# rcanut/nhwcodec

Hardware: AMD Instinct MI355X
Metric: encode Mpixels/s (512x512 RGB batch) (higher is better)
Workload: dtype int16

## Files before the change

### include/nhw_hip_debug.h

```cpp
#ifndef NHW_HIP_DEBUG_H
#define NHW_HIP_DEBUG_H

#include "nhw_hip.h"

#ifdef __cplusplus
extern "C" {
#endif

int nhw_debug_stop_after(nhw_enc *e, int stage);
int nhw_debug_front_fallback(nhw_enc *e, int on);
int nhw_debug_read(nhw_enc *e, int buf, int img, void *dst, size_t bytes);
int nhw_debug_hash(nhw_enc *e, int buf, size_t bytes, int n, void *d_out, void *stream);

int nhw_debug_fill(nhw_enc *e, int buf, int byte, size_t bytes, int n);

int nhw_debug_slice_order(nhw_enc *e, int mode);
int nhw_dec_debug_slice_order(nhw_dec *d, int mode);

int nhw_stage_chroma_loops(nhw_enc *e, int n, int comp, int form, void *stream);
int nhw_debug_write(nhw_enc *e, int buf, int img, const void *src, size_t bytes);

void nhw_dec_debug_stop_after(nhw_dec *d, int stage);
int  nhw_dec_debug_read(nhw_dec *d, int what, int img, void *dst, size_t bytes);
int  nhw_dec_debug_colour(int quality, const void *d_yuv, void *d_rgb, int n);

#ifdef __cplusplus
}
#endif
#endif
```

### nhwcodec_amd/__init__.py

```python
import ctypes
import numbers
import os

HERE = os.path.dirname(os.path.abspath(__file__))
LIB_PATH = os.path.join(HERE, "libnhwhip.so")
IMG_BYTES = 786432
OUT_STRIDE = 512 << 10
QUALITY_DEFAULT = 20
NHW_OK, NHW_E_QUALITY, NHW_E_CODEBOOK, NHW_E_SPACE, NHW_E_ARG, NHW_E_HIP, NHW_E_FORMAT = 0, -1, -2, -3, -4, -5, -6
NHW_E_BUDGET = -7
PEAK_SSE_NUMERATOR = 65025 * IMG_BYTES

P = ctypes.c_void_p


class Timing(ctypes.Structure):
    _fields_ = [(n, ctypes.c_float) for n in ("total_ms", "front_ms", "color_dwt_ms", "luma_ms", "chroma_ms", "entropy_ms")] + [("parts", ctypes.c_int), ("front_images", ctypes.c_int), ("prefilter_ms", ctypes.c_float)]


class FitStats(ctypes.Structure):
    _fields_ = [("rungs", ctypes.c_int), ("quality", ctypes.c_int * 23), ("images", ctypes.c_int * 23), ("total_ms", ctypes.c_float)]


class NhwError(RuntimeError):
# ... 10 lines not shown
    L.nhw_enc_create_ex.argtypes = [ctypes.c_int, ctypes.c_int, ctypes.c_uint, ctypes.POINTER(P)]
    L.nhw_enc_destroy.argtypes = [P]
    L.nhw_quality_supported.argtypes = [ctypes.c_int]
    L.nhw_enc_set_compat.argtypes = [P, ctypes.c_int]
    L.nhw_enc_batch_device.argtypes = [P, P, ctypes.c_int, ctypes.c_int, P, P, P, P]
    L.nhw_enc_batch.argtypes = [P, P, ctypes.c_int, ctypes.c_int, P, ctypes.c_size_t, P, P]
    L.nhw_synth_batch_device.argtypes = [P, P, ctypes.c_int, ctypes.c_uint32, P]
    L.nhw_enc_last_timing.argtypes = [P, ctypes.POINTER(Timing)]
    L.nhw_enc_synth_batch.argtypes = [P, ctypes.c_int, ctypes.c_uint32, ctypes.c_int, P, ctypes.c_size_t, P, P]
    L.nhw_host_alloc.restype = P
    L.nhw_host_alloc.argtypes = [ctypes.c_size_t]
    L.nhw_host_free.argtypes = [P]
    L.nhw_device_count.restype = ctypes.c_int
    L.nhw_enc_fit_batch_device.argtypes = [P, P, ctypes.c_int, P, P, ctypes.c_int, P, P, P, P, P]
    L.nhw_enc_fit_batch.argtypes = [P, P, ctypes.c_int, P, P, ctypes.c_int, P, ctypes.c_size_t, P, P, P]
    L.nhw_enc_last_fit_stats.argtypes = [P, ctypes.POINTER(FitStats)]
    L.nhw_sse_batch_device.argtypes = [P, P, ctypes.c_int, P, P]
    L.nhw_enc_fit_sse_batch_device.argtypes = [P, P, P, ctypes.c_int, P, P, ctypes.c_int, P, P, P, P, P, P]
    L.nhw_enc_fit_sse_batch.argtypes = [P, P, P, ctypes.c_int, P, P, ctypes.c_int, P, ctypes.c_size_t, P, P, P, P]
    L.nhw_stage_color.argtypes = [P, P, ctypes.c_int, ctypes.c_int, P, P, P, P]
    L.nhw_stage_prefilter.argtypes = [P, P, ctypes.c_int, ctypes.c_int, P]
    L.nhw_stage_chroma_l1.argtypes = [P, ctypes.c_int, P]
    L.nhw_stage_chroma_loops.argtypes = [P, ctypes.c_int, ctypes.c_int, ctypes.c_int, P]
    L.nhw_debug_write.argtypes = [P, ctypes.c_int, ctypes.c_int, P, ctypes.c_size_t]
    L.nhw_stage_analysis.argtypes = [P, P, P, ctypes.c_int, ctypes.c_size_t, ctypes.c_int, ctypes.c_int, ctypes.c_int, P]
    L.nhw_stage_synthesis.argtypes = [P, P, P, ctypes.c_int, ctypes.c_size_t, ctypes.c_int, ctypes.c_int, P]
    L.nhw_debug_slice_order.argtypes = [P, ctypes.c_int]
    L.nhw_dec_debug_slice_order.argtypes = [P, ctypes.c_int]
    L.nhw_picture_tiles.argtypes = [ctypes.c_uint32, ctypes.c_uint32]
    L.nhw_tile_pictures_device.argtypes = [P, ctypes.c_int, ctypes.c_int, ctypes.c_int, P, P]
    L.nhw_untile_pictures_device.argtypes = [P, P, ctypes.c_int, ctypes.c_int, ctypes.c_int, P]
    L.nhw_picture_info.argtypes = [P, ctypes.c_size_t, ctypes.POINTER(ctypes.c_uint32), ctypes.POINTER(ctypes.c_uint32)]
    L.nhw_enc_pictures.argtypes = [P, P, P, P, P, ctypes.c_int, ctypes.c_int, P, ctypes.c_size_t, P, P]
    L.nhw_dec_pictures.argtypes = [P, P, P, ctypes.c_int, P, P, P]
    L.nhw_sse_pictures_device.argtypes = [P, P, ctypes.c_int, ctypes.c_int, ctypes.c_int, P, P]
    L.nhw_enc_fit_pictures.argtypes = [P, P, P, P, P, ctypes.c_int, P, P, ctypes.c_int, P, ctypes.c_size_t, P, P, P]
    L.nhw_enc_fit_sse_pictures.argtypes = [P, P, P, P, P, P, ctypes.c_int, P, P, ctypes.c_int, P, ctypes.c_size_t, P, P, P, P]
    L.nhw_region_tiles.argtypes = [ctypes.c_uint32] * 6
    L.nhw_untile_regions_device.argtypes = [P, P, ctypes.c_int, ctypes.c_int, ctypes.c_int, P]
    L.nhw_dec_regions.argtypes = [P, P, P, ctypes.c_int, P, ctypes.c_int, P, P, P]
    L.nhw_dec_regions_to_device.argtypes = [P, P, P, ctypes.c_int, P, ctypes.c_int, P, P, P]
    L.nhw_dec_last_region_stats.argtypes = [P, ctypes.POINTER(ctypes.c_uint64), ctypes.POINTER(ctypes.c_uint64)]
    return L


_LIB = None
# ... 676 lines not shown
```

### nhwcodec_amd/csrc/nhw_dwt.h

```cpp
#ifndef NHW_DWT_H
#define NHW_DWT_H
#include <hip/hip_runtime.h>
#include <stdint.h>

__device__ __forceinline__ void lds_barrier() { asm volatile("s_waitcnt lgkmcnt(0)\n\ts_barrier" ::: "memory"); }

template <int S>
__device__ __forceinline__ void syn_pair(const int16_t *x, int st, int k, bool normalise, int *e_out, int *o_out)
{
	constexpr int M = S / 2;
	const int16_t *lo = x, *hi = x + M * st;
	const int l0 = lo[k * st], ln = (k + 1 < M) ? lo[(k + 1) * st] : l0;
	const int h0 = hi[k * st], hp = k > 0 ? hi[(k - 1) * st] : hi[0], hn = (k + 1 < M) ? hi[(k + 1) * st] : h0;
	int16_t e = (int16_t)(l0 << 3);
	int16_t o = (int16_t)((l0 + ln) << 2);
	e = (int16_t)(e - ((h0 + hp) << 1));
	o = (int16_t)(o + (6 * h0 - hp - hn));
	if (normalise) {
		if (e > 0) e = (int16_t)(e + 32);
		e >>= 6;
		if (o > 0) o = (int16_t)(o + 32);
		o >>= 6;
	}
	*e_out = e; *o_out = o;
// ... 29 lines not shown
typedef short s16x2 __attribute__((ext_vector_type(2)));
typedef unsigned short u16x2 __attribute__((ext_vector_type(2)));
__device__ __forceinline__ s16x2 as_s(uint32_t x) { return __builtin_bit_cast(s16x2, x); }
__device__ __forceinline__ u16x2 as_us(uint32_t x) { return __builtin_bit_cast(u16x2, x); }
__device__ __forceinline__ uint32_t as_w(s16x2 x) { return __builtin_bit_cast(uint32_t, x); }
__device__ __forceinline__ uint32_t as_w(u16x2 x) { return __builtin_bit_cast(uint32_t, x); }
__device__ __forceinline__ unsigned pk_add16(unsigned a, unsigned b)
{
	unsigned d;
	asm("v_pk_add_u16 %0, %1, %2" : "=v"(d) : "v"(a), "v"(b));
	return d;
}

__device__ __forceinline__ uint32_t pk_max_u16x(uint32_t a, uint32_t b) { uint32_t d; asm("v_pk_max_u16 %0, %1, %2" : "=v"(d) : "v"(a), "v"(b)); return d; }
__device__ __forceinline__ s16x2 pk_rnd_half_away(s16x2 v, int shift) { return (v + (s16x2)(short)(1 << (shift - 1)) + (v >> 15)) >> shift; }
__device__ __forceinline__ s16x2 pk_diffuse(s16x2 r)
{
	const s16x2 s = r >> 15, a = (r ^ s) - s;
	const s16x2 t = (s16x2)(a << 10) >> 10;
	const s16x2 d = (t + ((t >> 15) & (s16x2)(short)3)) >> 2;
	return (d ^ s) - s;
}

template <int PPL>
__device__ __forceinline__ void ana_row_pair(const uint32_t (&Dw)[PPL], int lane, int (&lo)[PPL], int (&hi)[PPL])
{
#pragma unroll
	for (int u = 0; u < PPL; u++) {
		uint32_t pv = (uint32_t)__builtin_amdgcn_update_dpp(0, (int)Dw[u], 0x138 , 0xF, 0xF, false);
		uint32_t nx = (uint32_t)__builtin_amdgcn_update_dpp(0, (int)Dw[u], 0x130 , 0xF, 0xF, false);
		if (u > 0) { const uint32_t seam = (uint32_t)__builtin_amdgcn_readlane((int)Dw[u > 0 ? u - 1 : 0], 63); if (lane == 0) pv = seam; }
		if (u + 1 < PPL) { const uint32_t seam = (uint32_t)__builtin_amdgcn_readlane((int)Dw[u + 1 < PPL ? u + 1 : u], 0); if (lane == 63) nx = seam; }
		else if (lane == 63) nx = Dw[u];
		const int e0 = (int16_t)(Dw[u] & 0xFFFF), o0 = (int)Dw[u] >> 16, e1 = (int16_t)(nx & 0xFFFF);
		int em1 = (int16_t)(pv & 0xFFFF), om1 = (int)pv >> 16;
		if (u == 0 && lane == 0) { em1 = e1; om1 = o0; }
		lo[u] = 6 * e0 + 2 * (om1 + o0) - (em1 + e1);
		hi[u] = (o0 << 1) - (e0 + e1);
	}
}

template <int PPL, int HLF, bool IN_RANGE = false >
__device__ __forceinline__ void ana_col_pair(const uint32_t (&Ew)[PPL], const uint32_t (&Ow)[PPL], bool left, int lane, int (&lo)[PPL][2], int (&hi)[PPL][2])
{
	bool wide = false;
	if (!IN_RANGE)
#pragma unroll
	for (int u = 0; u < PPL; u++) {
		const uint32_t mx = pk_max_u16x(pk_add16(Ew[u], 0x05140514u), pk_add16(Ow[u], 0x05140514u));
		wide |= (mx & 0xFFFFu) > 4300u || (mx >> 16) > 4300u;
	}
	if (IN_RANGE || !__any(wide)) {
		uint32_t rlast = 0;
#pragma unroll
		for (int u = 0; u < PPL; u++) {
			const int k = lane + 64 * u;
			uint32_t em = (uint32_t)__builtin_amdgcn_update_dpp(0, (int)Ew[u], 0x138, 0xF, 0xF, false), om = (uint32_t)__builtin_amdgcn_update_dpp(0, (int)Ow[u], 0x138, 0xF, 0xF, false);
			uint32_t en = (uint32_t)__builtin_amdgcn_update_dpp(0, (int)Ew[u], 0x130, 0xF, 0xF, false);
			if (u > 0) {
				const uint32_t se = (uint32_t)__builtin_amdgcn_readlane((int)Ew[u > 0 ? u - 1 : 0], 63), so_ = (uint32_t)__builtin_amdgcn_readlane((int)Ow[u > 0 ? u - 1 : 0], 63);
				if (lane == 0) { em = se; om = so_; }
			}
// ... 62 lines not shown
```

### nhwcodec_amd/csrc/nhw_enc.hip

```cpp
#include "nhw_enc.h"

thread_local std::string nhw_enc_err;
extern "C" const char *nhw_last_error(void) { return nhw_enc_err.c_str(); }

static const size_t k_buf_bytes[B_COUNT] = {
	 8 * Q,  8 * Q,  Q,  Q,  2 * Q,  2 * Q,
	 2 * Q,  2 * Q,  Q / 2,  Q / 2,  4 * Q,  2 * Q,
	 2 * Q,  4 * Q + 256,  8 * Q,  16,  512,  6 * Q,
	 24832,  16384,  16384 + 256,  32768,  16384,  32768,
	 8192,  2 * Q + 1024,  2 * Q + 256,  2 * Q + 1024,  2 * Q + 1024,  Q / 2,
	 Q + 64, 8192 + 64, 16384 + 64,  Q + 64, 8192 + 64, 16384 + 64,  Q + 64, 8192 + 64, 16384 + 64,
	 2 * Q + 1024, 16384 + 64, 16384 + 64,  2048 + 64,  8 * Q + 64,
	 512,  512,  320000,  768,  768,  16384 + 64,  16384 + 64,
	 131072,  131072,  5632,  256,  512,  16,  16,  (8 + 9 * 512) * 2,
	 Q / 2 + 256,  Q / 2,  Q / 4,  4 * Q,
	 Q / 4 + 256,  2 * Q,
	 2 * Q,  2 * Q,  Q / 2,  Q / 2,  Q,
	 320 * 512
};

static size_t round_up(size_t v, size_t a) { return (v + a - 1) / a * a; }

extern "C" int nhw_quality_supported(int quality) { return quality >= 1 && quality <= 23; }

// ... 119 lines not shown
	                    widen_in_analysis ? (comp ? plane8(ws, B_PV) : plane8(ws, B_PU)) : nullptr, ws.stride[B_PU], ws.dbg ? 0 : 2);
	if (low) nhw_launch_low_chroma_thin(cproc, cps, n, cs);
	STAGE_DONE();
	STAGE_DONE();
	if (!ws.dbg) {
		nhw_launch_chroma_loops(cproc, cps, cll1, ws.stride[B_CLL1] / 2, cl2save, ws.stride[B_CL2SAVE] / 2, plane8(ws, B_PU), ws.stride[B_PU], q, comp, ws.compat, n, cs);
		return 1;
	}
	nhw_launch_analysis(cjpeg, cproc, n, cps, H, H / 2, 1, cs);
	STAGE_DONE();
	nhw_launch_phase(PH_C2, ws, comp, out, d_sizes, d_status, cs);
	STAGE_DONE();
	nhw_launch_synthesis(cjpeg, cproc, n, cps, H, H / 2, cs);
	STAGE_DONE();
	nhw_launch_phase(PH_C3, ws, comp, out, d_sizes, d_status, cs);
	STAGE_DONE();
	nhw_launch_analysis(cjpeg, cproc, n, cps, H, H / 2, 1, cs, cl2save, ws.stride[B_CL2SAVE] / 2, H / 2, 1);
	STAGE_DONE();
	STAGE_DONE();
	nhw_launch_phase(PH_C4, ws, comp, out, d_sizes, d_status, cs);
	STAGE_DONE();
	nhw_launch_synthesis(cjpeg, cproc, n, cps, H, H / 2, cs);
	STAGE_DONE();
	return 1;
}

static int run_batch(nhw_enc *e, const NhwWs &ws_in, const void *d_bgr, int n, int quality, void *d_out, uint32_t *d_sizes, int32_t *d_status, hipStream_t s,
                     int timed ,
                     int what = 3 )
{
	NhwWs ws = ws_in;
	const int q = quality;
	const bool low = q <= 16;
	int16_t *jpeg = plane16(ws, B_JPEG), *proc = plane16(ws, B_PROC);
	int16_t *cjpeg = plane16(ws, B_CJPEG), *cproc = plane16(ws, B_CPROC);
	const size_t ps = ws.stride[B_JPEG] / 2, cps = ws.stride[B_CJPEG] / 2;
	uint8_t *out = (uint8_t *)d_out;

	e->low_parts_used = 1;
	int stage = 0;
	(void)n;
	if (what & 1) {
	if (timed == 1) HIPCHK(hipEventRecord(e->ev[EV_START], s));
	int16_t *yin = plane16(ws, B_KMAP);
	const size_t yin_stride = ws.stride[B_KMAP];
	if (low) {
// ... 23 lines not shown
	}
	STAGE_DONE();
	STAGE_DONE();
	if (timed == 1) HIPCHK(hipEventRecord(e->ev[EV_FRONT], s));
	if (!(what & 2)) { HIPCHK(hipGetLastError()); return NHW_OK; }
	}
	const bool fork = timed == 1 && what == 3 && !e->stop_after && e->chroma_fork;
	const bool fork_ll = fork && q > 13 && !ws.compat && e->ll_fork;
	ws.defer_verbatim = fork_ll;
	hipStream_t cs = fork ? e->part_stream[0] : s;
	ws.split_chroma = fork;
	auto chroma_head = [&](int comp) -> int { return chroma_head_launches(e, ws, comp, n, cs, stage); };
	auto chroma_tail = [&](int comp) -> int {
		nhw_launch_phase(PH_C5, ws, comp, out, d_sizes, d_status, cs);
		STAGE_DONE();
		return 1;
	};
#define CHROMA(call) do { const int rc_ = (call); if (rc_ != 1) return rc_; } while (0)
	if (fork) {
		HIPCHK(hipStreamWaitEvent(cs, !low || e->low_chroma == 0 ? e->ev[EV_FRONT] : (e->low_chroma == 2 && e->low_parts_used > 1) ? e->low_ev[low_ev_pass_a(e->low_parts_used - 1)] : e->ev[EV_COLOR], 0));
		CHROMA(chroma_head(0));
		CHROMA(chroma_head(1));
	}
	nhw_launch_analysis(jpeg, proc, n, ps, W, H, 1, s, nullptr, 0, 0, 0, nullptr, 0, 0, plane16(ws, B_LL1), ws.stride[B_LL1] / 2, H);
	STAGE_DONE();
	if (q > 6) {
	nhw_launch_phase(PH_L1, ws, 0, out, d_sizes, d_status, s);
	nhw_launch_wave(WV_DQ1, ws, s);
	STAGE_DONE();
	if (ws.dbg) {
	nhw_launch_synthesis(jpeg, proc, n, ps, W, H, s);
	STAGE_DONE();
	nhw_launch_phase(PH_L2, ws, 0, out, d_sizes, d_status, s);
	STAGE_DONE();
	} else nhw_launch_l2_recon(jpeg, proc, ps, plane16(ws, B_LL1), ws.stride[B_LL1] / 2, n, s);
	if (q > 12) nhw_launch_analysis(jpeg, proc, n, ps, W, H, 1, s, plane16(ws, B_L2SAVE), ws.stride[B_L2SAVE] / 2, H, 1);
	else nhw_launch_analysis(jpeg, proc, n, ps, W, H, 1, s);
	STAGE_DONE();
	}
	if (q <= 12) {
		nhw_launch_low_ll2(proc, ps, q, n, s);
		nhw_launch_copy_block(proc, ps, W, plane16(ws, B_L2SAVE), ws.stride[B_L2SAVE] / 2, H, H, H, n, s);
	}
	STAGE_DONE();
	nhw_launch_wave(WV_EMIT, ws, s);
	if (fork_ll) {
		HIPCHK(hipEventRecord(e->ll_ev[LL_EV_FORK], s));
		HIPCHK(hipStreamWaitEvent(e->ll_stream, e->ll_ev[LL_EV_FORK], 0));
		nhw_launch_phase(PH_L3, ws, 0, out, d_sizes, d_status, e->ll_stream);
		HIPCHK(hipEventRecord(e->ll_ev[LL_EV_DONE], e->ll_stream));
		HIPCHK(hipEventRecord(e->part_ev[PE_LUMA_LIST], e->ll_stream));
	} else {
	nhw_launch_phase(PH_L3, ws, 0, out, d_sizes, d_status, s);
	if (fork) HIPCHK(hipEventRecord(e->part_ev[PE_LUMA_LIST], s));
	}
	if (q > 12) {
	nhw_launch_wave(WV_DQ0, ws, s);
	STAGE_DONE();
	if (fork_ll) {
		HIPCHK(hipStreamWaitEvent(s, e->ll_ev[LL_EV_DONE], 0));
		nhw_launch_synthesis(jpeg, proc, n, ps, W, H, s, q <= 21 && !ws.dbg, ws.buf<uint16_t>(B_LLMEM, 0), ws.stride[B_LLMEM], &ws.buf<NhwMeta>(B_META, 0)->ll_mem_len, ws.stride[B_META]);
	} else
// ... 217 lines not shown
	HIPCHK(hipStreamWaitEvent(s, e->ev[EV_END], 0));
	int16_t *cjpeg = plane16(ws, B_CJPEG), *cproc = plane16(ws, B_CPROC), *cll1 = plane16(ws, B_CLL1), *cl2save = plane16(ws, B_CL2SAVE);
	const size_t cps = ws.stride[B_CJPEG] / 2;
	if (form == 0) {
		int stage = 0;
		const int rc = chroma_head_launches(e, ws, comp, n, s, stage);
		if (rc != 1) return rc;
	} else if (form == 1)
		nhw_launch_chroma_loops(cproc, cps, cll1, ws.stride[B_CLL1] / 2, cl2save, ws.stride[B_CL2SAVE] / 2, plane8(ws, B_PU), ws.stride[B_PU], ws.q, comp, ws.compat, n, s);
	else {
		const int k = form - 1;
		nhw_launch_analysis(cjpeg, cproc, n, cps, H, H / 2, 1, s, nullptr, 0, 0, 0, nullptr, 0, 0, cll1, ws.stride[B_CLL1] / 2, H / 2);
		if (k > 1) nhw_launch_phase(PH_C2, ws, comp, nullptr, nullptr, nullptr, s);
		if (k > 2) nhw_launch_synthesis(cjpeg, cproc, n, cps, H, H / 2, s);
		if (k > 3) nhw_launch_phase(PH_C3, ws, comp, nullptr, nullptr, nullptr, s);
		if (k > 4) nhw_launch_analysis(cjpeg, cproc, n, cps, H, H / 2, 1, s, cl2save, ws.stride[B_CL2SAVE] / 2, H / 2, 1);
		if (k > 5) nhw_launch_phase(PH_C4, ws, comp, nullptr, nullptr, nullptr, s);
		if (k > 6) nhw_launch_synthesis(cjpeg, cproc, n, cps, H, H / 2, s);
	}
	HIPCHK(hipGetLastError());
	return NHW_OK;
}

extern "C" int nhw_stage_synthesis(nhw_enc *e, void *d_jpeg, void *d_proc, int n_img, size_t plane_stride, int stride, int size, void *stream)
{
	if (!e || n_img < 1) return NHW_E_ARG;
	if (size != 256 && size != 128) { nhw_enc_err = "synthesis: transform size must be 256 or 128 (the encoder has no synthesis of size 512)"; return NHW_E_ARG; }
	HIPCHK(hipSetDevice(e->device));
	nhw_launch_synthesis((int16_t *)d_jpeg, (int16_t *)d_proc, n_img, plane_stride, stride, size, stream ? (hipStream_t)stream : e->own_stream);
	HIPCHK(hipGetLastError());
	return NHW_OK;
}

extern "C" int nhw_debug_front_fallback(nhw_enc *e, int on) { if (!e) return NHW_E_ARG; e->front_fallback = on; return NHW_OK; }
extern "C" int nhw_debug_stop_after(nhw_enc *e, int stage) { if (!e) return NHW_E_ARG; e->stop_after = stage; return NHW_OK; }
extern "C" int nhw_debug_slice_order(nhw_enc *e, int mode) { if (!e || mode < 0 || mode > 2) return NHW_E_ARG; e->slice_order = mode; return NHW_OK; }
__global__ __launch_bounds__(256) void k_debug_hash(const uint8_t *base, size_t stride, size_t words, unsigned long long *out)
{
	const uint32_t *p = reinterpret_cast<const uint32_t *>(base + (size_t)blockIdx.x * stride);
	unsigned long long h = 0;
	for (size_t i = threadIdx.x; i < words; i += 256) {
		unsigned long long x = ((unsigned long long)p[i] + 0x9E3779B97F4A7C15ull) * (2 * i + 1);
		x ^= x >> 29; x *= 0xBF58476D1CE4E5B9ull; x ^= x >> 32;
		h += x;
	}
	if (threadIdx.x == 0) out[blockIdx.x] = 0;
// ... 37 lines not shown
```

### nhwcodec_amd/csrc/nhw_host.h

```cpp
#ifndef NHW_HOST_H
#define NHW_HOST_H

#include <hip/hip_runtime.h>
#include <stdint.h>
#include <string>
#include <vector>

#include "../../include/nhw_hip.h"

struct NhwWs;

extern thread_local int nhw_slice_mode;

struct NhwSliceScope {
	int saved;
	explicit NhwSliceScope(int mode) : saved(nhw_slice_mode) { nhw_slice_mode = mode; }
	~NhwSliceScope() { nhw_slice_mode = saved; }
};

template <typename F> inline void nhw_slices(int nslices, F &&launch)
{
	if (nhw_slice_mode == 1) for (int i = 0; i < nslices; i++) launch(i);
	else if (nhw_slice_mode == 2) for (int i = nslices - 1; i >= 0; i--) launch(i);
	else launch(-1);
}

void nhw_launch_color(const uint8_t *bgr, int n, int q, int16_t *y, size_t y_stride, uint8_t *u, uint8_t *v, size_t c_stride, hipStream_t s);
void nhw_launch_analysis(int16_t *jpeg, int16_t *proc, int n, size_t plane_stride, int stride, int size, int final_level, hipStream_t s,
                         int16_t *save = nullptr, size_t save_plane = 0, int save_row = 0, int save_kind = 0, const uint8_t *src8 = nullptr, size_t src8_plane = 0, int drop_t = 0,
                         const int16_t *alt = nullptr, size_t alt_plane = 0, int alt_stride = 0);
void nhw_launch_synthesis(int16_t *jpeg, int16_t *proc, int n, size_t plane_stride, int stride, int size, hipStream_t s, int drop_nat = 0,
                          const uint16_t *verb_list = nullptr, size_t verb_list_stride = 0, const int *verb_len = nullptr, size_t verb_len_stride = 0);
void nhw_launch_synth(uint8_t *bgr, int n, uint32_t seed_base, hipStream_t s);
void nhw_launch_front_fused(const uint8_t *bgr, int q, uint8_t *pu, uint8_t *pv, size_t c_stride, const int16_t *y, size_t y_stride, int with_prefilter,
                            uint8_t *st, size_t s_stride, int16_t *proc, int16_t *jpeg, size_t plane_stride, int16_t *ll1, size_t ll1_stride,
                            int16_t *keep, size_t keep_stride, int n, hipStream_t s, int switches);
void nhw_launch_front_stale(const int16_t *y, size_t y_stride, const uint8_t *st, size_t s_stride, int16_t *stale, size_t stale_stride, int n, hipStream_t s);
int nhw_front_set_attrs(const char **where);
enum { PH_L1, PH_L2, PH_L3, PH_L4A, PH_C0, PH_C2, PH_C3, PH_C4, PH_C5, PH_FINAL, PH_L4B, PH_L4C, PH_L4D, PH_LLC, PH_L4C2 };
enum { WV_DQ1, WV_DQ0, WV_EMIT, WV_QUANT };
void nhw_launch_phase(int ph, const NhwWs &ws, int comp, uint8_t *out, uint32_t *sizes, int32_t *status, hipStream_t s);
void nhw_launch_wave(int ph, const NhwWs &ws, hipStream_t s);
void nhw_launch_l2_recon(int16_t *jpeg, const int16_t *proc, size_t plane_stride, int16_t *ll1, size_t ll1_stride, int n, hipStream_t s);
void nhw_launch_chroma_loops(int16_t *cproc, size_t plane_stride, int16_t *cll1, size_t ll1_stride, int16_t *cl2save, size_t save_stride,
                             const uint8_t *pu, size_t pu_stride, int q, int comp, int compat, int n, hipStream_t s);
void nhw_launch_copy_block(const int16_t *src, size_t src_plane, int src_row, int16_t *dst, size_t dst_plane, int dst_row, int rows, int cols, int n, hipStream_t s);
int nhw_tail_set_attrs(const char **where);
enum { LOW_EV_START = 0, LOW_EV_COUNT = 13 };
inline int low_ev_pass_a(int p) { return 1 + p; }
inline int low_ev_done(int parts, int p) { return 1 + parts + p; }
int nhw_launch_low_prefilter(const int16_t *src, size_t src_stride, int16_t *y, size_t y_stride, int16_t *km, size_t km_stride, uint8_t *so, size_t so_stride, uint8_t *chain, size_t chain_stride,
                             uint16_t *tab, size_t tab_stride, int q, int n, hipStream_t s, int force = 0, int parts = 1, hipStream_t *aux = nullptr, hipEvent_t *ev = nullptr);
void nhw_launch_low_prefilter_chroma(const uint8_t *src, size_t src_stride, int16_t *dst, size_t dst_stride, int q, int n, hipStream_t s);
void nhw_launch_low_chroma_thin(int16_t *plane, size_t plane_stride, int n, hipStream_t s);
void nhw_launch_low_ll2(int16_t *proc, size_t plane_stride, int q, int n, hipStream_t s);
void nhw_launch_low_stale(const int16_t *km, size_t km_stride, int16_t *stale, size_t stale_stride, int n, hipStream_t s);
void nhw_launch_fit_gather(const uint8_t *d_bgr, const int *idx, int m, uint8_t *staging, hipStream_t s);
void nhw_launch_fit_select(const int *idx, int m, const uint8_t *st_out, const uint32_t *st_sizes, const int32_t *st_status, const void *limit,
                           const int32_t *dec_status, const uint64_t *sse, int quality, int last, uint8_t *out, uint32_t *sizes, int32_t *status,
                           int32_t *qual, uint64_t *sse_out, uint8_t *open, hipStream_t s);
void nhw_launch_fit_compact(const uint8_t *open, const int *idx, int m, int *next, int *count, hipStream_t s);
hipError_t nhw_launch_sse(const uint8_t *a, const uint8_t *b, int n, uint64_t *sse, hipStream_t s);
hipError_t nhw_launch_tile_pad(const nhw_picture *d_pics, int n_pics, int tile0, int m, uint8_t *d_tiles, hipStream_t s);
hipError_t nhw_launch_untile_crop(const uint8_t *d_tiles, const nhw_picture *d_pics, int n_pics, int tile0, int m, hipStream_t s);
hipError_t nhw_launch_untile_region(const uint8_t *d_tiles, const nhw_region *d_regs, int n_regs, int tile0, int m, hipStream_t s);
hipError_t nhw_launch_sse_crop(const uint8_t *d_tiles, const nhw_picture *d_pics, int n_pics, int tile0, int m, uint64_t *d_sse, hipStream_t s);
// ... 22 lines not shown
```

### nhwcodec_amd/csrc/nhw_tail.hip

```cpp
#include "nhw_host.h"
#include "nhw_tail_par.h"
#include "nhw_dwt.h"

using namespace nhw;

#ifndef NHW_DENSE_STREAM
#define NHW_DENSE_STREAM 0
#endif

template <int PH>
__global__ __launch_bounds__(256) void k_phase(NhwWs ws, int comp, uint8_t *out, uint32_t *sizes, int32_t *status)
{
	__shared__ int sh_counts[2];
	__shared__ int sh_pos[2 * NT + 2];
	__shared__ uint32_t sh_z[4 * Q / 16 / 32 + 4];
	extern __shared__ __attribute__((aligned(16))) int16_t dyn_lds[];
	const int img = blockIdx.x, tid = threadIdx.x;
	Ctx c;
	ctx_load(&c, ws, img, comp);
	if (PH == PH_L1) luma_p1_par(&c, tid, sh_pos);
	else if (PH == PH_L2) luma_p2_par(&c, tid, dyn_lds);
	else if (PH == PH_L3) luma_p3_par(&c, tid, sh_pos, sh_counts, dyn_lds, ws.q <= 12 || ws.dbg != 0);
	else if (PH == PH_L4A) luma_p4a_par(&c, tid, dyn_lds);
	else if (PH == PH_L4B) luma_p4b_par(&c, tid, sh_pos, dyn_lds);
// ... 52 lines not shown
	if (img >= ws.n) return;
	Ctx c;
	ctx_load(&c, ws, img);
	if (PH == WV_DQ1) wave_dequant_sim_luma(&c, 1, lane, dq_lut, false, ws.dbg != 0);
	else if (PH == WV_DQ0) wave_dequant_sim_luma(&c, 0, lane, dq_lut, !ws.dbg, ws.dbg != 0);
	else if (PH == WV_QUANT) {
		__shared__ __attribute__((aligned(16))) uint8_t park[4][16 * QROW];
		__shared__ uint32_t lut[4][QLUT + 3];
		PROF_BEGIN(); wave_quantise_luma(&c, lane, park[threadIdx.x >> 6], lut[threadIdx.x >> 6], ws.q > 21 || ws.dbg, NHW_DENSE_STREAM || ws.dbg, !(ws.q > 21 || ws.dbg)); if (!lane) PROF(&c, 15);
	}
	else if (PH == WV_EMIT) { PROF_BEGIN(); wave_emit_ll2(&c, lane); if (!lane) PROF(&c, 4); }
}
void nhw_launch_wave(int ph, const NhwWs &ws, hipStream_t s)
{
	const dim3 g((ws.n + 3) / 4), b(256);
	switch (ph) {
	case WV_DQ1: k_wave<WV_DQ1><<<g, b, 0, s>>>(ws); break;
	case WV_DQ0: k_wave<WV_DQ0><<<g, b, 0, s>>>(ws); break;
	case WV_EMIT: k_wave<WV_EMIT><<<g, b, 0, s>>>(ws); break;
	case WV_QUANT: k_wave<WV_QUANT><<<g, b, 0, s>>>(ws); break;
	}
}

__global__ __launch_bounds__(1024) void k_l2_recon(int16_t *__restrict__ jpegb, const int16_t *__restrict__ procb, size_t plane_stride, int16_t *__restrict__ ll1b, size_t ll1_stride, int n)
{
	extern __shared__ __attribute__((aligned(16))) int16_t smem[];
	constexpr int S = H, LS = S + 2, HLF = S / 2, PPL = HLF / 64, NT_ = 1024, NPRE = S * (S / 8) / NT_;
	const int t = threadIdx.x, lane = t & 63, wv = t >> 6;
	int16_t *A = smem;
	int8_t *ytab = reinterpret_cast<int8_t *>(A + S * LS);
	if (t < PRECOMP_TAB) ytab[t] = (int8_t)precomp_pick(t / 11 - 12, t % 11 - 5);
	uint4 pre[NPRE];
	if ((int)blockIdx.x < n) {
		const int16_t *src = jpegb + (size_t)blockIdx.x * plane_stride;
#pragma unroll
		for (int u = 0; u < NPRE; u++) { const int v = t + u * NT_; pre[u] = *reinterpret_cast<const uint4 *>(src + (size_t)(v / (S / 8)) * W + 8 * (v % (S / 8))); }
	}
	for (int img = blockIdx.x; img < n; img += gridDim.x) {
		int16_t *jp = jpegb + (size_t)img * plane_stride, *o = ll1b + (size_t)img * ll1_stride;
		const int16_t *p = procb + (size_t)img * plane_stride;
#pragma unroll
		for (int u = 0; u < NPRE; u++) {
			const int v = t + u * NT_, row = v / (S / 8), c8 = v % (S / 8);
			uint32_t *d = reinterpret_cast<uint32_t *>(A + row * LS + 8 * c8);
			d[0] = pre[u].x; d[1] = pre[u].y; d[2] = pre[u].z; d[3] = pre[u].w;
		}
		lds_barrier();
		if (img + (int)gridDim.x < n) {
			const int16_t *src = jpegb + (size_t)(img + gridDim.x) * plane_stride;
#pragma unroll
			for (int u = 0; u < NPRE; u++) { const int v = t + u * NT_; pre[u] = *reinterpret_cast<const uint4 *>(src + (size_t)(v / (S / 8)) * W + 8 * (v % (S / 8))); }
		}
		const int r0 = wv * 16, c0 = 4 * lane;
		int side = 0;
		if (lane < 16) side = p[(size_t)(r0 + lane) * W - 1];
		else if (lane < 32) side = p[(size_t)(r0 + lane - 16) * W + H];
		else if (lane == 32) { side = o[(size_t)r0 * H - 1]; if (wv > 0) side = side > 14000 ? side - 16000 : side > 10000 ? side - 12000 : side; }
		else if (lane == 33) { side = o[(size_t)(r0 + 16) * H]; if (wv < 15) side = side > 14000 ? side - 16000 : side > 10000 ? side - 12000 : side; }
		for (int i = 0; i < 16; i++) {
			int16_t *x = A + (wv * 16 + i) * LS;
			int e[PPL], od[PPL];
#pragma unroll
			for (int u = 0; u < PPL; u++) syn_pair<S>(x, 1, lane + 64 * u, false, &e[u], &od[u]);
#pragma unroll
			for (int u = 0; u < PPL; u++) reinterpret_cast<uint32_t *>(x)[lane + 64 * u] = (uint32_t)(uint16_t)e[u] | ((uint32_t)(uint16_t)od[u] << 16);
		}
		lds_barrier();
		for (int i = 0; i < 16; i++) {
			int16_t *x = A + wv * 16 + i;
			int e[PPL], od[PPL];
#pragma unroll
			for (int u = 0; u < PPL; u++) syn_pair<S>(x, LS, lane + 64 * u, true, &e[u], &od[u]);
#pragma unroll
			for (int u = 0; u < PPL; u++) { const int k = lane + 64 * u; x[(2 * k) * LS] = (int16_t)e[u]; x[(2 * k + 1) * LS] = (int16_t)od[u]; }
		}
		lds_barrier();
		auto ll1_row = [&](int i) { return *reinterpret_cast<const uint2 *>(o + (size_t)(r0 + (i < 16 ? i : 15)) * H + c0); };
		auto untag = [](int v) { return v > 14000 ? v - 16000 : v > 10000 ? v - 12000 : v; };
		uint2 w0 = ll1_row(0), w1 = ll1_row(1), w2 = ll1_row(2), w3 = ll1_row(3);
#pragma unroll 1
		for (int i = 0; i < 16; i++) {
			const int r = r0 + i;
			int v[4];
			unpack4(w0, v);
			w0 = w1; w1 = w2; w2 = w3; w3 = ll1_row(i + 4);
			bool any = false;
#pragma unroll
			for (int k = 0; k < 4; k++) {
				const int step = v[k] > 14000 ? 1 : v[k] > 10000 ? -1 : 0;
				if (!step) continue;
// ... 21 lines not shown
			const int o_right = i == 15 ? __builtin_amdgcn_readlane(side, 33) : untag((int)(int16_t)(__builtin_amdgcn_readlane((int)w1.x, 0) & 0xFFFF));
			w0 = w1; w1 = w2; w2 = w3; w3 = ll1_row(i + 4);
#pragma unroll
			for (int k = 0; k < 4; k++) { ov[k] = untag(ov[k]); pv[k] = A[(c0 + k) * LS + r]; d[k] = (int16_t)(pv[k] - ov[k]); }
			const int p_left = __shfl(side, i), p_right = __shfl(side, 16 + i);
			const int my_edge = lane ? p_right - o_right : p_left - o_left;
			o_left = __builtin_amdgcn_readlane(ov[3], 63);
			const int sd = __shfl_down(d[0], 1), su = __shfl_up(d[3], 1);
			const int dn4 = lane < 63 ? sd : my_edge;
			const int first = lane ? su : my_edge;
			const int nb[4] = { precomp_right(d[1]), precomp_right(d[2]), precomp_right(d[3]), precomp_right(dn4) };
			int prev_in = first;
			for (;;) {
				int prev = prev_in;
#pragma unroll
				for (int k = 0; k < 4; k++) { st[k] = ytab[precomp_index(d[k], nb[k] + prev)]; prev = d[k] + st[k]; }
				int np = __shfl_up(prev, 1);
				if (!lane) np = first;
				if (!__any(np != prev_in)) break;
				prev_in = np;
			}
			uint2 w;
			w.x = (uint32_t)(uint16_t)(ov[0] + st[0]) | ((uint32_t)(uint16_t)(ov[1] + st[1]) << 16); w.y = (uint32_t)(uint16_t)(ov[2] + st[2]) | ((uint32_t)(uint16_t)(ov[3] + st[3]) << 16);
			*reinterpret_cast<uint2 *>(jp + (size_t)r * W + c0) = w;
		}
		lds_barrier();
	}
}
void nhw_launch_l2_recon(int16_t *jpeg, const int16_t *proc, size_t plane_stride, int16_t *ll1, size_t ll1_stride, int n, hipStream_t s)
{
	k_l2_recon<<<n < 256 ? n : 256, 1024, H * (H + 2) * sizeof(int16_t) + 288, s>>>(jpeg, proc, plane_stride, ll1, ll1_stride, n);
}

__global__ __launch_bounds__(512) __attribute__((amdgpu_waves_per_eu(8, 8))) void k_chroma_loops(int16_t *__restrict__ cprocb, size_t plane_stride, int16_t *__restrict__ cll1b, size_t ll1_stride,
                                                      int16_t *__restrict__ saveb, size_t save_stride, const uint8_t *__restrict__ pub, size_t pu_stride,
                                                      int q, int comp, int compat)
{
	constexpr int S = H / 2, LS = S + 2, HLF = S / 2;
	__shared__ __attribute__((aligned(16))) int16_t A[S * LS];
	const int t = threadIdx.x, lane = t & 63, wv = t >> 6, img = blockIdx.x, r0 = wv * 16;
	int16_t *p = cprocb + (size_t)img * plane_stride, *o = cll1b + (size_t)img * ll1_stride, *save = saveb + (size_t)img * save_stride;
	const uint8_t *pu = pub + (size_t)img * pu_stride;
	const int behind = compat ? (int16_t)(pu[32768] | (pu[32769] << 8)) : 0;
	auto ll1_row = [&](int i) { return reinterpret_cast<const uint32_t *>(o + (size_t)(r0 + (i < 16 ? i : 15)) * S)[lane]; };
	uint32_t w0 = ll1_row(0), w1 = ll1_row(1), w2 = ll1_row(2), w3 = ll1_row(3);
	int side = 0;
	if (lane < 16) side = p[(size_t)(r0 + lane) * H + S];
	else if (lane == 16) side = wv < 7 ? o[(size_t)(r0 + 16) * S] : behind;
	if (t == 0) o[Q >> 2] = (int16_t)behind;
	auto ana_row = [&](int16_t *x, uint32_t w) {
		const uint32_t Dw[1] = { w };
		int lo[1], hi[1];
		ana_row_pair<1>(Dw, lane, lo, hi);
		x[lane] = (int16_t)lo[0]; x[HLF + lane] = (int16_t)hi[0];
// ... 111 lines not shown

static size_t phase_lds(int ph)
{
	const size_t tile = (size_t)NT * TLS * sizeof(int16_t);
	switch (ph) {
	case PH_L2: return 3 * 32 * 33 + 32;
	case PH_L3: return LL_LDS_BYTES;
	case PH_LLC: return LLC_LDS_BYTES;
	case PH_FINAL: return PK_LDS_BYTES;
	case PH_L4A: return RF_LDS_BYTES > (NT + 2) * TLS * sizeof(int16_t) ? RF_LDS_BYTES : (size_t)(NT + 2) * TLS * sizeof(int16_t);
	case PH_L4B: return (size_t)(NT + 2) * TLS * sizeof(int16_t);
	case PH_L4C: return 0;
	case PH_L4D: return SL_LDS_BYTES;
	case PH_C5: return CQ_LDS_BYTES > 32 * 130 * 2 + (32 * 128 + 258) * 2 ? CQ_LDS_BYTES : 32 * 130 * 2 + (32 * 128 + 258) * 2;
	default: return 0;
	}
}

int nhw_tail_set_attrs(const char **where)
{
#define SETATTR(fn) do { const hipError_t e_ = hipFuncSetAttribute(reinterpret_cast<const void *>(&fn), hipFuncAttributeMaxDynamicSharedMemorySize, 100 << 10); \
                         if (e_ != hipSuccess) { *where = "hipFuncSetAttribute(" #fn ", MaxDynamicSharedMemorySize)"; return (int)e_; } } while (0)
	SETATTR(k_phase<PH_L1>); SETATTR(k_phase<PH_L2>); SETATTR(k_phase<PH_L3>); SETATTR(k_phase<PH_C5>);
	{ const hipError_t e_ = hipFuncSetAttribute(reinterpret_cast<const void *>(&k_l2_recon), hipFuncAttributeMaxDynamicSharedMemorySize, (int)(H * (H + 2) * sizeof(int16_t) + 288));
	  if (e_ != hipSuccess) { *where = "hipFuncSetAttribute(k_l2_recon, MaxDynamicSharedMemorySize)"; return (int)e_; } }
#undef SETATTR
	return 0;
}

void nhw_launch_phase(int ph, const NhwWs &ws, int comp, uint8_t *out, uint32_t *sizes, int32_t *status, hipStream_t s)
{
	const dim3 g(ws.n), b(256);
	const size_t lds = phase_lds(ph);
	switch (ph) {
	case PH_L1: k_phase<PH_L1><<<g, b, lds, s>>>(ws, comp, out, sizes, status); break;
	case PH_L2: k_phase<PH_L2><<<g, b, lds, s>>>(ws, comp, out, sizes, status); break;
	case PH_L3: k_phase<PH_L3><<<g, b, lds, s>>>(ws, comp, out, sizes, status); break;
	case PH_L4A: if (ws.q >= 17) k_l4a<<<g, b, lds, s>>>(ws); else k_phase<PH_L4A><<<g, b, lds, s>>>(ws, comp, out, sizes, status); break;
	case PH_L4B: k_phase<PH_L4B><<<g, b, lds, s>>>(ws, comp, out, sizes, status); break;
	case PH_L4C: k_phase<PH_L4C><<<g, b, lds, s>>>(ws, comp, out, sizes, status); break;
	case PH_L4D: if (NHW_DENSE_STREAM || ws.dbg) k_phase<PH_L4D><<<g, b, lds, s>>>(ws, comp, out, sizes, status); else k_y31<<<g, 512, lds, s>>>(ws); break;
	case PH_LLC: k_phase<PH_LLC><<<g, b, lds, s>>>(ws, comp, out, sizes, status); break;
	case PH_L4C2: k_phase<PH_L4C2><<<g, b, lds, s>>>(ws, comp, out, sizes, status); break;
	case PH_C0: k_phase<PH_C0><<<g, b, lds, s>>>(ws, comp, out, sizes, status); break;
	case PH_C2: k_phase<PH_C2><<<g, b, lds, s>>>(ws, comp, out, sizes, status); break;
	case PH_C3: k_phase<PH_C3><<<g, b, lds, s>>>(ws, comp, out, sizes, status); break;
	case PH_C4: k_phase<PH_C4><<<g, b, lds, s>>>(ws, comp, out, sizes, status); break;
	case PH_C5: k_phase<PH_C5><<<g, b, lds, s>>>(ws, comp, out, sizes, status); break;
// ... 11 lines not shown
```

Baseline: 60820.

## Fuse level-2 luma analysis into l2_recon kernel for high quality

For quality above 12, the L2 reconstruction kernel now also runs the level-1 row and column analysis on the reconstructed plane while it is still in LDS. It writes jpeg, proc and the L2 save buffer directly, so the separate analysis launch and its global-memory round trip are removed. Row analysis uses DPP lane shifts to get neighbouring pixels. The luma loop launch sequence moves into a helper, and a new stage entry point is added to benchmark variants. The change adds LDS work and barriers inside the recon kernel, and adds an unroll pragma to the inner synthesis loop.

```diff
diff --git a/include/nhw_hip_debug.h b/include/nhw_hip_debug.h
--- a/include/nhw_hip_debug.h
+++ b/include/nhw_hip_debug.h
@@ -19,6 +19,7 @@
 
 int nhw_stage_chroma_loops(nhw_enc *e, int n, int comp, int form, void *stream);
 int nhw_debug_write(nhw_enc *e, int buf, int img, const void *src, size_t bytes);
+int nhw_stage_luma_loop(nhw_enc *e, int n, int form, void *stream);
 
 void nhw_dec_debug_stop_after(nhw_dec *d, int stage);
 int  nhw_dec_debug_read(nhw_dec *d, int what, int img, void *dst, size_t bytes);
diff --git a/nhwcodec_amd/__init__.py b/nhwcodec_amd/__init__.py
--- a/nhwcodec_amd/__init__.py
+++ b/nhwcodec_amd/__init__.py
@@ -56,6 +56,7 @@
     L.nhw_stage_prefilter.argtypes = [P, P, ctypes.c_int, ctypes.c_int, P]
     L.nhw_stage_chroma_l1.argtypes = [P, ctypes.c_int, P]
     L.nhw_stage_chroma_loops.argtypes = [P, ctypes.c_int, ctypes.c_int, ctypes.c_int, P]
+    L.nhw_stage_luma_loop.argtypes = [P, ctypes.c_int, ctypes.c_int, P]
     L.nhw_debug_write.argtypes = [P, ctypes.c_int, ctypes.c_int, P, ctypes.c_size_t]
     L.nhw_stage_analysis.argtypes = [P, P, P, ctypes.c_int, ctypes.c_size_t, ctypes.c_int, ctypes.c_int, ctypes.c_int, P]
     L.nhw_stage_synthesis.argtypes = [P, P, P, ctypes.c_int, ctypes.c_size_t, ctypes.c_int, ctypes.c_int, P]
diff --git a/nhwcodec_amd/csrc/nhw_dwt.h b/nhwcodec_amd/csrc/nhw_dwt.h
--- a/nhwcodec_amd/csrc/nhw_dwt.h
+++ b/nhwcodec_amd/csrc/nhw_dwt.h
@@ -75,6 +75,15 @@
 	return (d ^ s) - s;
 }
 
+__device__ __forceinline__ void ana_row_taps(uint32_t d, uint32_t pv, uint32_t nx, bool first, int *lo, int *hi)
+{
+	const int e0 = (int16_t)(d & 0xFFFF), o0 = (int)d >> 16, e1 = (int16_t)(nx & 0xFFFF);
+	int em1 = (int16_t)(pv & 0xFFFF), om1 = (int)pv >> 16;
+	if (first) { em1 = e1; om1 = o0; }
+	*lo = 6 * e0 + 2 * (om1 + o0) - (em1 + e1);
+	*hi = (o0 << 1) - (e0 + e1);
+}
+
 template <int PPL>
 __device__ __forceinline__ void ana_row_pair(const uint32_t (&Dw)[PPL], int lane, int (&lo)[PPL], int (&hi)[PPL])
 {
@@ -85,12 +94,17 @@
 		if (u > 0) { const uint32_t seam = (uint32_t)__builtin_amdgcn_readlane((int)Dw[u > 0 ? u - 1 : 0], 63); if (lane == 0) pv = seam; }
 		if (u + 1 < PPL) { const uint32_t seam = (uint32_t)__builtin_amdgcn_readlane((int)Dw[u + 1 < PPL ? u + 1 : u], 0); if (lane == 63) nx = seam; }
 		else if (lane == 63) nx = Dw[u];
-		const int e0 = (int16_t)(Dw[u] & 0xFFFF), o0 = (int)Dw[u] >> 16, e1 = (int16_t)(nx & 0xFFFF);
-		int em1 = (int16_t)(pv & 0xFFFF), om1 = (int)pv >> 16;
-		if (u == 0 && lane == 0) { em1 = e1; om1 = o0; }
-		lo[u] = 6 * e0 + 2 * (om1 + o0) - (em1 + e1);
-		hi[u] = (o0 << 1) - (e0 + e1);
+		ana_row_taps(Dw[u], pv, nx, u == 0 && lane == 0, &lo[u], &hi[u]);
 	}
+}
+
+__device__ __forceinline__ void ana_row_quad(uint32_t a, uint32_t b, int lane, int (&lo)[2], int (&hi)[2])
+{
+	const uint32_t pv = (uint32_t)__builtin_amdgcn_update_dpp(0, (int)b, 0x138 , 0xF, 0xF, false);
+	uint32_t nx = (uint32_t)__builtin_amdgcn_update_dpp(0, (int)a, 0x130 , 0xF, 0xF, false);
+	if (lane == 63) nx = b;
+	ana_row_taps(a, pv, b, lane == 0, &lo[0], &hi[0]);
+	ana_row_taps(b, a, nx, false, &lo[1], &hi[1]);
 }
 
 template <int PPL, int HLF, bool IN_RANGE = false >
diff --git a/nhwcodec_amd/csrc/nhw_enc.hip b/nhwcodec_amd/csrc/nhw_enc.hip
--- a/nhwcodec_amd/csrc/nhw_enc.hip
+++ b/nhwcodec_amd/csrc/nhw_enc.hip
@@ -165,6 +165,32 @@
 	STAGE_DONE();
 	nhw_launch_synthesis(cjpeg, cproc, n, cps, H, H / 2, cs);
 	STAGE_DONE();
+	return 1;
+}
+
+static int luma_loop_launches(nhw_enc *e, const NhwWs &ws, int n, hipStream_t s, int &stage)
+{
+	const int q = ws.q;
+	int16_t *jpeg = plane16(ws, B_JPEG), *proc = plane16(ws, B_PROC);
+	const size_t ps = ws.stride[B_JPEG] / 2;
+	uint8_t *out = nullptr; uint32_t *d_sizes = nullptr; int32_t *d_status = nullptr;
+	nhw_launch_analysis(jpeg, proc, n, ps, W, H, 1, s, nullptr, 0, 0, 0, nullptr, 0, 0, plane16(ws, B_LL1), ws.stride[B_LL1] / 2, H);
+	STAGE_DONE();
+	if (q > 6) {
+	nhw_launch_phase(PH_L1, ws, 0, out, d_sizes, d_status, s);
+	nhw_launch_wave(WV_DQ1, ws, s);
+	STAGE_DONE();
+	if (ws.dbg) {
+	nhw_launch_synthesis(jpeg, proc, n, ps, W, H, s);
+	STAGE_DONE();
+	nhw_launch_phase(PH_L2, ws, 0, out, d_sizes, d_status, s);
+	STAGE_DONE();
+	} else nhw_launch_l2_recon(jpeg, proc, ps, plane16(ws, B_LL1), ws.stride[B_LL1] / 2, n, s,
+	                           q > 12 ? plane16(ws, B_L2SAVE) : nullptr, ws.stride[B_L2SAVE] / 2);
+	if (q <= 12) nhw_launch_analysis(jpeg, proc, n, ps, W, H, 1, s);
+	else if (ws.dbg) nhw_launch_analysis(jpeg, proc, n, ps, W, H, 1, s, plane16(ws, B_L2SAVE), ws.stride[B_L2SAVE] / 2, H, 1);
+	STAGE_DONE();
+	}
 	return 1;
 }
 
@@ -234,22 +260,7 @@
 		CHROMA(chroma_head(0));
 		CHROMA(chroma_head(1));
 	}
-	nhw_launch_analysis(jpeg, proc, n, ps, W, H, 1, s, nullptr, 0, 0, 0, nullptr, 0, 0, plane16(ws, B_LL1), ws.stride[B_LL1] / 2, H);
-	STAGE_DONE();
-	if (q > 6) {
-	nhw_launch_phase(PH_L1, ws, 0, out, d_sizes, d_status, s);
-	nhw_launch_wave(WV_DQ1, ws, s);
-	STAGE_DONE();
-	if (ws.dbg) {
-	nhw_launch_synthesis(jpeg, proc, n, ps, W, H, s);
-	STAGE_DONE();
-	nhw_launch_phase(PH_L2, ws, 0, out, d_sizes, d_status, s);
-	STAGE_DONE();
-	} else nhw_launch_l2_recon(jpeg, proc, ps, plane16(ws, B_LL1), ws.stride[B_LL1] / 2, n, s);
-	if (q > 12) nhw_launch_analysis(jpeg, proc, n, ps, W, H, 1, s, plane16(ws, B_L2SAVE), ws.stride[B_L2SAVE] / 2, H, 1);
-	else nhw_launch_analysis(jpeg, proc, n, ps, W, H, 1, s);
-	STAGE_DONE();
-	}
+	{ const int rc_ = luma_loop_launches(e, ws, n, s, stage); if (rc_ != 1) return rc_; }
 	if (q <= 12) {
 		nhw_launch_low_ll2(proc, ps, q, n, s);
 		nhw_launch_copy_block(proc, ps, W, plane16(ws, B_L2SAVE), ws.stride[B_L2SAVE] / 2, H, H, H, n, s);
@@ -513,6 +524,45 @@
 	return NHW_OK;
 }
 
+extern "C" int nhw_stage_luma_loop(nhw_enc *e, int n, int form, void *stream)
+{
+	if (!e || n < 1 || n > e->max_batch || form < 0 || form > 5) { nhw_enc_err = "bad argument"; return NHW_E_ARG; }
+	if (!e->timed || n > e->last_n || e->stop_after || e->last_q < 7) {
+		nhw_enc_err = "nhw_stage_luma_loop: needs a completed whole batch of >= n images at quality >= 7 and no debug stop";
+		return NHW_E_ARG;
+	}
+	HIPCHK(hipSetDevice(e->device));
+	NhwWs ws = e->ws;
+	ws.n = n; ws.q = e->last_q; ws.dbg = 0;
+	hipStream_t s = stream ? (hipStream_t)stream : e->own_stream;
+	HIPCHK(hipStreamWaitEvent(s, e->ev[EV_END], 0));
+	int16_t *jpeg = plane16(ws, B_JPEG), *proc = plane16(ws, B_PROC), *ll1 = plane16(ws, B_LL1), *l2save = plane16(ws, B_L2SAVE);
+	const size_t ps = ws.stride[B_JPEG] / 2;
+	const bool save = ws.q > 12;
+	if (form == 0) {
+		int stage = 0;
+		const int rc = luma_loop_launches(e, ws, n, s, stage);
+		if (rc != 1) return rc;
+	} else if (form == 1) {
+		nhw_launch_l2_recon(jpeg, proc, ps, ll1, ws.stride[B_LL1] / 2, n, s, save ? l2save : nullptr, ws.stride[B_L2SAVE] / 2);
+		if (!save) nhw_launch_analysis(jpeg, proc, n, ps, W, H, 1, s);
+	} else {
+		if (form == 3 || form == 4) {
+			nhw_launch_analysis(jpeg, proc, n, ps, W, H, 1, s, nullptr, 0, 0, 0, nullptr, 0, 0, ll1, ws.stride[B_LL1] / 2, H);
+			nhw_launch_phase(PH_L1, ws, 0, nullptr, nullptr, nullptr, s);
+			nhw_launch_wave(WV_DQ1, ws, s);
+		}
+		nhw_launch_synthesis(jpeg, proc, n, ps, W, H, s);
+		if (form < 4) {
+			nhw_launch_phase(PH_L2, ws, 0, nullptr, nullptr, nullptr, s);
+			if (save) nhw_launch_analysis(jpeg, proc, n, ps, W, H, 1, s, l2save, ws.stride[B_L2SAVE] / 2, H, 1);
+			else nhw_launch_analysis(jpeg, proc, n, ps, W, H, 1, s);
+		}
+	}
+	HIPCHK(hipGetLastError());
+	return NHW_OK;
+}
+
 extern "C" int nhw_stage_synthesis(nhw_enc *e, void *d_jpeg, void *d_proc, int n_img, size_t plane_stride, int stride, int size, void *stream)
 {
 	if (!e || n_img < 1) return NHW_E_ARG;
diff --git a/nhwcodec_amd/csrc/nhw_host.h b/nhwcodec_amd/csrc/nhw_host.h
--- a/nhwcodec_amd/csrc/nhw_host.h
+++ b/nhwcodec_amd/csrc/nhw_host.h
@@ -41,7 +41,7 @@
 enum { WV_DQ1, WV_DQ0, WV_EMIT, WV_QUANT };
 void nhw_launch_phase(int ph, const NhwWs &ws, int comp, uint8_t *out, uint32_t *sizes, int32_t *status, hipStream_t s);
 void nhw_launch_wave(int ph, const NhwWs &ws, hipStream_t s);
-void nhw_launch_l2_recon(int16_t *jpeg, const int16_t *proc, size_t plane_stride, int16_t *ll1, size_t ll1_stride, int n, hipStream_t s);
+void nhw_launch_l2_recon(int16_t *jpeg, int16_t *proc, size_t plane_stride, int16_t *ll1, size_t ll1_stride, int n, hipStream_t s, int16_t *l2save = nullptr, size_t save_stride = 0);
 void nhw_launch_chroma_loops(int16_t *cproc, size_t plane_stride, int16_t *cll1, size_t ll1_stride, int16_t *cl2save, size_t save_stride,
                              const uint8_t *pu, size_t pu_stride, int q, int comp, int compat, int n, hipStream_t s);
 void nhw_launch_copy_block(const int16_t *src, size_t src_plane, int src_row, int16_t *dst, size_t dst_plane, int dst_row, int rows, int cols, int n, hipStream_t s);
diff --git a/nhwcodec_amd/csrc/nhw_tail.hip b/nhwcodec_amd/csrc/nhw_tail.hip
--- a/nhwcodec_amd/csrc/nhw_tail.hip
+++ b/nhwcodec_amd/csrc/nhw_tail.hip
@@ -98,7 +98,9 @@
 	}
 }
 
-__global__ __launch_bounds__(1024) void k_l2_recon(int16_t *__restrict__ jpegb, const int16_t *__restrict__ procb, size_t plane_stride, int16_t *__restrict__ ll1b, size_t ll1_stride, int n)
+template <bool ANA>
+__global__ __launch_bounds__(1024) void k_l2_recon(int16_t *__restrict__ jpegb, int16_t *__restrict__ procb, size_t plane_stride, int16_t *__restrict__ ll1b, size_t ll1_stride, int n,
+                                                   int16_t *__restrict__ saveb, size_t save_stride)
 {
 	extern __shared__ __attribute__((aligned(16))) int16_t smem[];
 	constexpr int S = H, LS = S + 2, HLF = S / 2, PPL = HLF / 64, NT_ = 1024, NPRE = S * (S / 8) / NT_;
@@ -114,7 +116,7 @@
 	}
 	for (int img = blockIdx.x; img < n; img += gridDim.x) {
 		int16_t *jp = jpegb + (size_t)img * plane_stride, *o = ll1b + (size_t)img * ll1_stride;
-		const int16_t *p = procb + (size_t)img * plane_stride;
+		int16_t *p = procb + (size_t)img * plane_stride;
 #pragma unroll
 		for (int u = 0; u < NPRE; u++) {
 			const int v = t + u * NT_, row = v / (S / 8), c8 = v % (S / 8);
@@ -142,6 +144,7 @@
 			for (int u = 0; u < PPL; u++) reinterpret_cast<uint32_t *>(x)[lane + 64 * u] = (uint32_t)(uint16_t)e[u] | ((uint32_t)(uint16_t)od[u] << 16);
 		}
 		lds_barrier();
+#pragma unroll 4
 		for (int i = 0; i < 16; i++) {
 			int16_t *x = A + wv * 16 + i;
 			int e[PPL], od[PPL];
@@ -209,14 +212,52 @@
 			}
 			uint2 w;
 			w.x = (uint32_t)(uint16_t)(ov[0] + st[0]) | ((uint32_t)(uint16_t)(ov[1] + st[1]) << 16); w.y = (uint32_t)(uint16_t)(ov[2] + st[2]) | ((uint32_t)(uint16_t)(ov[3] + st[3]) << 16);
-			*reinterpret_cast<uint2 *>(jp + (size_t)r * W + c0) = w;
+			if (!ANA) *reinterpret_cast<uint2 *>(jp + (size_t)r * W + c0) = w;
+			else {
+				int lo[2], hi[2];
+				ana_row_quad(w.x, w.y, lane, lo, hi);
+				int16_t *x = A + (2 * lane) * LS + r;
+				x[0] = (int16_t)lo[0]; x[LS] = (int16_t)lo[1]; x[HLF * LS] = (int16_t)hi[0]; x[(HLF + 1) * LS] = (int16_t)hi[1];
+			}
+		}
+		if (ANA) {
+			lds_barrier();
+			int16_t *save = saveb + (size_t)img * save_stride;
+			const int rr = lane >> 5, c8 = lane & 31;
+#pragma unroll 1
+			for (int i = 0; i < 8; i++) {
+				const int c = r0 + 2 * i;
+				const uint32_t *g = reinterpret_cast<const uint32_t *>(A + (c + rr) * LS + 8 * c8);
+				*reinterpret_cast<uint4 *>(jp + (size_t)(c + rr) * W + 8 * c8) = make_uint4(g[0], g[1], g[2], g[3]);
+				uint32_t Ew[PPL], Ow[PPL];
+				int lo[PPL][2], hi[PPL][2];
+#pragma unroll
+				for (int u = 0; u < PPL; u++) {
+					const uint32_t a = reinterpret_cast<const uint32_t *>(A + c * LS)[lane + 64 * u], b = reinterpret_cast<const uint32_t *>(A + (c + 1) * LS)[lane + 64 * u];
+					Ew[u] = (a & 0xFFFFu) | (b << 16); Ow[u] = (a >> 16) | (b & 0xFFFF0000u);
+				}
+				ana_col_pair<PPL, HLF>(Ew, Ow, c < HLF, lane, lo, hi);
+				asm volatile("" ::: "memory");
+#pragma unroll
+				for (int h = 0; h < 2; h++) {
+					int16_t *x = A + (c + h) * LS;
+#pragma unroll
+					for (int u = 0; u < PPL; u++) { x[lane + 64 * u] = (int16_t)lo[u][h]; x[HLF + lane + 64 * u] = (int16_t)hi[u][h]; }
+				}
+				asm volatile("" ::: "memory");
+				const uint4 w = make_uint4(g[0], g[1], g[2], g[3]);
+				*reinterpret_cast<uint4 *>(p + (size_t)(c + rr) * W + 8 * c8) = w;
+				*reinterpret_cast<uint4 *>(save + (size_t)(c + rr) * H + 8 * c8) = w;
+			}
 		}
 		lds_barrier();
 	}
 }
-void nhw_launch_l2_recon(int16_t *jpeg, const int16_t *proc, size_t plane_stride, int16_t *ll1, size_t ll1_stride, int n, hipStream_t s)
-{
-	k_l2_recon<<<n < 256 ? n : 256, 1024, H * (H + 2) * sizeof(int16_t) + 288, s>>>(jpeg, proc, plane_stride, ll1, ll1_stride, n);
+void nhw_launch_l2_recon(int16_t *jpeg, int16_t *proc, size_t plane_stride, int16_t *ll1, size_t ll1_stride, int n, hipStream_t s,
+                         int16_t *l2save , size_t save_stride)
+{
+	if (l2save) k_l2_recon<true><<<n < 256 ? n : 256, 1024, H * (H + 2) * sizeof(int16_t) + 288, s>>>(jpeg, proc, plane_stride, ll1, ll1_stride, n, l2save, save_stride);
+	else k_l2_recon<false><<<n < 256 ? n : 256, 1024, H * (H + 2) * sizeof(int16_t) + 288, s>>>(jpeg, proc, plane_stride, ll1, ll1_stride, n, nullptr, 0);
 }
 
 __global__ __launch_bounds__(512) __attribute__((amdgpu_waves_per_eu(8, 8))) void k_chroma_loops(int16_t *__restrict__ cprocb, size_t plane_stride, int16_t *__restrict__ cll1b, size_t ll1_stride,
@@ -374,8 +415,10 @@
 #define SETATTR(fn) do { const hipError_t e_ = hipFuncSetAttribute(reinterpret_cast<const void *>(&fn), hipFuncAttributeMaxDynamicSharedMemorySize, 100 << 10); \
                          if (e_ != hipSuccess) { *where = "hipFuncSetAttribute(" #fn ", MaxDynamicSharedMemorySize)"; return (int)e_; } } while (0)
 	SETATTR(k_phase<PH_L1>); SETATTR(k_phase<PH_L2>); SETATTR(k_phase<PH_L3>); SETATTR(k_phase<PH_C5>);
-	{ const hipError_t e_ = hipFuncSetAttribute(reinterpret_cast<const void *>(&k_l2_recon), hipFuncAttributeMaxDynamicSharedMemorySize, (int)(H * (H + 2) * sizeof(int16_t) + 288));
-	  if (e_ != hipSuccess) { *where = "hipFuncSetAttribute(k_l2_recon, MaxDynamicSharedMemorySize)"; return (int)e_; } }
+	for (const void *fn : { reinterpret_cast<const void *>(&k_l2_recon<false>), reinterpret_cast<const void *>(&k_l2_recon<true>) }) {
+		const hipError_t e_ = hipFuncSetAttribute(fn, hipFuncAttributeMaxDynamicSharedMemorySize, (int)(H * (H + 2) * sizeof(int16_t) + 288));
+		if (e_ != hipSuccess) { *where = "hipFuncSetAttribute(k_l2_recon, MaxDynamicSharedMemorySize)"; return (int)e_; }
+	}
 #undef SETATTR
 	return 0;
 }
```

Measured after the change: 62160 (median of 6 runs). 1.02x the previous value.
